# Guanys-dar/GM-Diffusion

Measured on AMD Instinct MI355X. Metric: HDR images/sec @ 512x512, 50 PNDM steps, dual-UNet, higher is better.
Workload: dtype bf16; 1 GPU; SD-v1-5 dual-UNet (SDR 4ch + GM 8ch) 512x512, 50 PNDM steps (51 iterations), CFG 7.5, batch 4/GPU, 2 VAE decodes + Eq.1 HDR tail; global_batch=4, per_gpu_batch=4, resolution=512, inference_steps=50, parallelism=prompt-batch sharding x1, RCCL broadcast of text hidden states + latents

## Files before the change

gm-diffusion_amd/csrc/attention.hip:

```cpp
#include "gmd_common.h"

#include <type_traits>

int gmd_launch_attention_split(const void* Q, const void* K, const void* Vt, void* O, int B, int H, int D, int Nq, int Nk, int64_t ldq,
                               int64_t ldk, int64_t ldvt, int64_t ldo, int64_t sQ, int64_t sK, int64_t sVt, int64_t sO, float scale, int o_split,
                               hipStream_t stream);

namespace {

struct AttnParams {
    const bf16_t* Q;
    const bf16_t* K;
    const bf16_t* Vt;
    bf16_t* O;
    int Nq, Nk, H;
    int64_t ldq, ldk, ldvt, ldo, sQ, sK, sVt, sO;
    float scale_log2;
};

typedef unsigned int u32x4 __attribute__((ext_vector_type(4)));

constexpr int KV = 64;
constexpr int VROW = 136;
constexpr float kNegBig = -1.0e30f;

template <typename HT, int D, bool CAUSAL>
__global__ __launch_bounds__(256, D <= 40 ? 4 : (D <= 64 ? 3 : 1)) void attn_fwd_kernel(const AttnParams p) {
    GMD_WG_TRACE_SCOPE(WGK_ATTN);
    constexpr int DK = (D + 15) / 16;
    constexpr int DT = (D + 31) / 32;
    constexpr int KROW = (2 * DK + 1) * 16;
    constexpr int DC = D / 8;
    static_assert(D % 8 == 0, "head dim must be a multiple of 8");
    extern __shared__ __attribute__((aligned(16))) unsigned char smem[];
    constexpr int kStageBytes = KV * KROW + DT * 32 * VROW;
    constexpr int NKC = (KV * DC + 255) / 256;
    constexpr int NVC = (D * 8 + 255) / 256;
    constexpr bool kRowSumMfma = DT * 32 > D;
    constexpr bool kLagged = kRowSumMfma && DK * 16 > D;
    constexpr float kLagMax = std::is_same<HT, f16_t>::value ? 14.0f : 20.0f;

    const int tid = threadIdx.x, lane = tid & 63, wid = tid >> 6;
    const int r = lane & 31, hh = lane >> 5;
    int qb, head, b;
    {
        const int nwg = gridDim.x, id = blockIdx.x;
        const int qq = nwg >> 3, rr = nwg & 7, xcd = id & 7, j = id >> 3;
        const int L = (xcd < rr ? xcd * (qq + 1) : rr * (qq + 1) + (xcd - rr) * qq) + j;
        const int nqb = (p.Nq + 127) / 128;
        qb = L % nqb;
        const int t = L / nqb;
        head = t % p.H;
        b = t / p.H;
    }
// ... 270 lines not shown
        for (int kt = 0; kt < ntiles; kt += 2) {
            tile(kt, std::integral_constant<int, 0>{}, std::false_type{});
            if (kt + 1 < ntiles) tile(kt + 1, std::integral_constant<int, 1>{}, std::false_type{});
        }
    }

    float l_tot;
    if constexpr (kRowSumMfma) {
        l_tot = __shfl(ot[D / 32][4 * ((D % 32) / 8)], r, 64);
    } else {
        l_tot = half_swap_sum(l_run);
    }
    const float inv = 1.0f / l_tot;
    constexpr int SROW = D * 2 + 16;
    unsigned char* strip = smem + wid * (32 * SROW);
#pragma unroll
    for (int dt = 0; dt < DT; ++dt)
#pragma unroll
        for (int g = 0; g < 4; ++g) {
            const int d0 = 32 * dt + 8 * g + 4 * hh;
            if (d0 < D) {
                uint2 w;
                w.x = Half<HT>::pack2(ot[dt][4 * g + 0] * inv, ot[dt][4 * g + 1] * inv);
                w.y = Half<HT>::pack2(ot[dt][4 * g + 2] * inv, ot[dt][4 * g + 3] * inv);
                *reinterpret_cast<uint2*>(strip + r * SROW + d0 * 2) = w;
            }
        }
    __builtin_amdgcn_wave_barrier();
    constexpr int CH = D / 8;
    const int q0w = qb * 128 + wid * 32;
    bf16_t* Ow = p.O + (int64_t)b * p.sO + (int64_t)q0w * p.ldo + (int64_t)head * D;
#pragma unroll
    for (int t = 0; t < (32 * CH + 63) / 64; ++t) {
        const int idx = lane + 64 * t;
        const int rr = idx / CH, cc = idx - rr * CH;
        if (rr < 32 && q0w + rr < p.Nq)
            *reinterpret_cast<uint4*>(Ow + (int64_t)rr * p.ldo + cc * 8) = *reinterpret_cast<const uint4*>(strip + rr * SROW + cc * 16);
    }
}

template <int N> __device__ __forceinline__ void attn_wait_vmcnt() { asm volatile("s_waitcnt vmcnt(%0)" ::"n"(N) : "memory"); }

#if defined(GMD_ATTN40_PRIO) && GMD_ATTN40_PRIO == 1
#define ATTN40_PRIO_MFMA(x) __builtin_amdgcn_s_setprio(x);
#define ATTN40_PRIO_VALU(x)
#elif defined(GMD_ATTN40_PRIO) && GMD_ATTN40_PRIO == 2
#define ATTN40_PRIO_MFMA(x)
#define ATTN40_PRIO_VALU(x) __builtin_amdgcn_s_setprio(x);
#else
#define ATTN40_PRIO_MFMA(x)
#define ATTN40_PRIO_VALU(x)
#endif
template <typename HT>
__global__ __launch_bounds__(256, 4) void attn40_kernel(const AttnParams p) {
    GMD_WG_TRACE_SCOPE(WGK_ATTN40);
    constexpr int D = 40, DK = 3, DT = 2, NST = 3;
    constexpr int KROWB = 2 * D;
    constexpr int kLagOff = KV * KROWB;
    constexpr int kVOff = 5376;
    constexpr int kStage = kVOff + (D + 2) * 128;
    static_assert(kLagOff + 16 <= kVOff && kStage % 256 == 0, "stage layout");
    constexpr float kLagMax = std::is_same<HT, f16_t>::value ? 14.0f : 20.0f;
    extern __shared__ __attribute__((aligned(16))) unsigned char smem[];

    const int tid = threadIdx.x, lane = tid & 63, wid = tid >> 6;
    const int wuni = __builtin_amdgcn_readfirstlane(wid);
    const int r = lane & 31, hh = lane >> 5;
    int qb, head, b;
    {
        const int nwg = gridDim.x, id = blockIdx.x;
        const int qq = nwg >> 3, rr = nwg & 7, xcd = id & 7, j = id >> 3;
        const int L = (xcd < rr ? xcd * (qq + 1) : rr * (qq + 1) + (xcd - rr) * qq) + j;
        const int nqb = (p.Nq + 127) / 128;
        qb = L % nqb;
        const int t = L / nqb;
        head = t % p.H;
        b = t / p.H;
    }
    const int q = qb * 128 + wid * 32 + r;
    const bool qvalid = q < p.Nq;
    const bf16_t* Qb = p.Q + (int64_t)b * p.sQ + (int64_t)head * D;
    const bf16_t* Kb = p.K + (int64_t)b * p.sK + (int64_t)head * D;
    const bf16_t* Vb = p.Vt + (int64_t)b * p.sVt + (int64_t)head * D * p.ldvt;

    for (int i = tid; i < NST * 24; i += 256) {
        const int st = i / 24, e = i - st * 24;
        unsigned char* base = smem + st * kStage;
        if (e < 8) {
            const unsigned one2 = Half<HT>::kOne | (Half<HT>::kOne << 16);
            *reinterpret_cast<uint4*>(base + kVOff + D * 128 + e * 16) = make_uint4(one2, one2, one2, one2);
        } else if (e < 16) {
            *reinterpret_cast<uint4*>(base + kVOff + (D + 1) * 128 + (e - 8) * 16) = make_uint4(0, 0, 0, 0);
        } else if (e == 16) {
            *reinterpret_cast<uint4*>(base + kLagOff) = make_uint4(Half<HT>::kOne, 0, 0, 0);
        }
    }

    uint4 qf[DK];
#pragma unroll
    for (int s = 0; s < DK; ++s) {
        const int d0 = 16 * s + 8 * hh;
        uint4 v = make_uint4(0, 0, 0, 0);
        if (qvalid && d0 + 8 <= D) v = *reinterpret_cast<const uint4*>(Qb + (int64_t)q * p.ldq + d0);
        unsigned w[4] = {v.x, v.y, v.z, v.w};
#pragma unroll
        for (int j = 0; j < 4; ++j) {
            float lo, hi;
// ... 211 lines not shown
                }
            }
            mx = half_swap_max(mx);
            set_stabiliser(Half<HT>::round(mx));
        }
        for (int kt = 0; kt < ntiles; kt += 3) {
            tile(kt, std::integral_constant<int, 0>{}, lag_c);
            if (kt + 1 < ntiles) tile(kt + 1, std::integral_constant<int, 1>{}, lag_c);
            if (kt + 2 < ntiles) tile(kt + 2, std::integral_constant<int, 2>{}, lag_c);
        }
    };
    run(std::true_type{});
    if (__syncthreads_or(lag_overflow)) {
#pragma unroll
        for (int t = 0; t < DT; ++t)
#pragma unroll
            for (int i = 0; i < 16; ++i) ot[t][i] = 0.f;
        set_stabiliser(0.f);
        m_run = kNegBig;
        run(std::false_type{});
        __syncthreads();
    }

    const float l_tot = __shfl(ot[1][4], r, 64);
    const float inv = 1.0f / l_tot;
    constexpr int SROW = D * 2 + 16;
    unsigned char* strip = smem + wid * (32 * SROW);
#pragma unroll
    for (int dt = 0; dt < DT; ++dt)
#pragma unroll
        for (int g = 0; g < 4; ++g) {
            const int d0 = 32 * dt + 8 * g + 4 * hh;
            if (d0 < D) {
                uint2 w;
                w.x = Half<HT>::pack2(ot[dt][4 * g + 0] * inv, ot[dt][4 * g + 1] * inv);
                w.y = Half<HT>::pack2(ot[dt][4 * g + 2] * inv, ot[dt][4 * g + 3] * inv);
                *reinterpret_cast<uint2*>(strip + r * SROW + d0 * 2) = w;
            }
        }
    __builtin_amdgcn_wave_barrier();
    constexpr int CH = D / 8;
    const int q0w = qb * 128 + wid * 32;
    bf16_t* Ow = p.O + (int64_t)b * p.sO + (int64_t)q0w * p.ldo + (int64_t)head * D;
#pragma unroll
    for (int t = 0; t < (32 * CH + 63) / 64; ++t) {
        const int idx = lane + 64 * t;
        const int rr = idx / CH, cc = idx - rr * CH;
        if (rr < 32 && q0w + rr < p.Nq)
            *reinterpret_cast<uint4*>(Ow + (int64_t)rr * p.ldo + cc * 8) = *reinterpret_cast<const uint4*>(strip + rr * SROW + cc * 16);
    }
}

template <typename HT>
int launch_attn40(const AttnParams& p, int B, int H, hipStream_t s) {
    constexpr size_t smem = 3 * (5376 + 42 * 128);
    dim3 grid(((p.Nq + 127) / 128) * H * B, 1, 1);
    attn40_kernel<HT><<<grid, 256, smem, s>>>(p);
    hipError_t e = hipGetLastError();
    if (e != hipSuccess) {
        gmd_set_error("gmd_attention: launch failed: %s", hipGetErrorString(e));
        return GMD_ERR_LAUNCH;
    }
    return GMD_OK;
}

template <typename HT, int D, bool CAUSAL = false>
int launch_attn(const AttnParams& p, int B, int H, hipStream_t s) {
    constexpr int DK = (D + 15) / 16, DT = (D + 31) / 32;
    const size_t smem = 2 * ((size_t)KV * (2 * DK + 1) * 16 + (size_t)DT * 32 * VROW);
    dim3 grid(((p.Nq + 127) / 128) * H * B, 1, 1);
    attn_fwd_kernel<HT, D, CAUSAL><<<grid, 256, smem, s>>>(p);
    hipError_t e = hipGetLastError();
    if (e != hipSuccess) {
        gmd_set_error("gmd_attention: launch failed: %s", hipGetErrorString(e));
        return GMD_ERR_LAUNCH;
    }
    return GMD_OK;
}

template <typename HT>
int dispatch_attn(const AttnParams& p, int B, int H, int D, int Nq, int Nk, int causal, hipStream_t s) {
    if (causal) {
        GMD_REQUIRE(Nq == Nk, "gmd_attention: the causal mask needs Nq == Nk");
        if (D == 64) return launch_attn<HT, 64, true>(p, B, H, s);
        if (D == 32) return launch_attn<HT, 32, true>(p, B, H, s);
        gmd_set_error("gmd_attention: causal attention is instantiated for head dims 32 and 64 only (got %d)", D);
        return GMD_ERR_UNSUPPORTED;
    }
    switch (D) {
        case 32: return launch_attn<HT, 32>(p, B, H, s);
        case 40: return launch_attn40<HT>(p, B, H, s);
        case 64: return launch_attn<HT, 64>(p, B, H, s);
        case 80: return launch_attn<HT, 80>(p, B, H, s);
        case 160: return launch_attn<HT, 160>(p, B, H, s);
        default:
            gmd_set_error("gmd_attention: head dim %d not instantiated (supported: 32, 40, 64, 80, 160)", D);
            return GMD_ERR_UNSUPPORTED;
    }
}

}

extern "C" int gmd_attention(const void* Q, const void* K, const void* Vt, void* O, int dtype, int B, int H, int D, int Nq,
                             int Nk, int64_t ldq, int64_t ldk, int64_t ldvt, int64_t ldo, int64_t strideQ, int64_t strideK,
                             int64_t strideVt, int64_t strideO, float scale, int causal, gmd_stream_t stream) {
    if (dtype == GMD_F32S || dtype == GMD_F32SA) {
        GMD_REQUIRE(!causal, "gmd_attention: the float32 (split) kernel has no causal mask");
        GMD_REQUIRE(B >= 0 && H > 0 && Nq >= 0 && Nk > 0, "gmd_attention: bad shape B=%d H=%d Nq=%d Nk=%d", B, H, Nq, Nk);
        if (B == 0 || Nq == 0) return GMD_OK;
        GMD_REQUIRE((int64_t)((Nq + 127) / 128) * H * B < (1ll << 31), "gmd_attention: grid too large");
// ... 37 lines not shown
```

gm-diffusion_amd/csrc/gemm.hip:

```cpp
#include "gemm_shared.h"
#include <stdlib.h>
#include <type_traits>

int gmd_launch_split_gemm(const void* params, int presplit, int batch, void* ws, int64_t ws_bytes, hipStream_t s, const char* name);
int gmd_launch_split_conv(const void* params, int presplit, int B, void* ws, int64_t ws_bytes, hipStream_t s, const char* name);
int gmd_split_plan_ksplit(int M, int N, int K, int64_t ws_bytes);
int gmd_split_colstats_ok(int M, int N, int K, int batch, int64_t ws_bytes, int bucket);
int gmd_split_out_ok(int M, int N, int K, int geglu, int64_t ws_bytes);
int gmd_split_qkv_vt_ok(int M, int N, int K, int vt_col0, int vt_tokens, int64_t ws_bytes);
void gmd_split_set_lc(int mode);

namespace {

template <typename HT>
__device__ __forceinline__ void epilogue_store8(const GemmParams& p, int z, int m, int n, float (&v)[8]) {
    const bool vec_ok = (p.ldc % 8 == 0) && (p.sC % 8 == 0) && (p.residual == nullptr || (p.ldr % 8 == 0 && p.sR % 8 == 0));
    const int nvalid = p.N - n < 8 ? p.N - n : 8;
    const float* rb = p.rowbias ? p.rowbias + (int64_t)(m / p.rows_per_group) * p.ldrb : nullptr;
    const HT* res = p.residual ? (const HT*)p.residual + (int64_t)z * p.sR + (int64_t)m * p.ldr + n : nullptr;
    float rv[8];
    if (res) {
        if (nvalid == 8 && vec_ok) load_vec(res, rv);
        else
            for (int j = 0; j < 8; ++j) rv[j] = j < nvalid ? Elem<HT>::ld(res + j) : 0.f;
// ... 882 lines not shown
            wait_tiles(rem < D - 1 ? rem : D - 1);
            __syncthreads();
            if (kt + D < nk) dma_tile(kt + D, st_fill);
            compute(st_cur);
            st_cur = st_cur + 1 == NST ? 0 : st_cur + 1;
            st_fill = st_fill + 1 == NST ? 0 : st_fill + 1;
        }
    }
    const bool rows_ok = !p.out_f32 && p.ksplit <= 1 && p.act != GMD_ACT_GEGLU && m0 + BM <= p.M && n0 + BN <= p.N && (p.ldc & 7) == 0 &&
                         (p.sC & 7) == 0 && (p.residual == nullptr || ((p.ldr & 7) == 0 && (p.sR & 7) == 0)) &&
                         (p.rowbias == nullptr || ((p.ldrb & 3) == 0 && (reinterpret_cast<uintptr_t>(p.rowbias) & 15) == 0)) &&
                         (reinterpret_cast<uintptr_t>(p.bias) & 15) == 0;
    if constexpr (TN % 2 == 0) {
        if (p.act == GMD_ACT_GEGLU && !p.out_f32 && p.ksplit <= 1 && m0 + BM <= p.M && n0 + BN <= p.N && (p.ldc & 7) == 0 && (p.sC & 7) == 0 &&
            (reinterpret_cast<uintptr_t>(p.bias) & 15) == 0) {
            __syncthreads();
            constexpr int kStripG = 32 * (TN * 8 + 4);
            epilogue_rows_geglu<HT, TM, TN>(p, acc, reinterpret_cast<float*>(smem) + wid * kStripG, m0 + wr * 64, n0 + wc * (TN * 16), lane, z);
            return;
        }
    }
    if (p.ksplit > 1 && m0 + BM <= p.M && n0 + BN <= p.N && (p.N & 3) == 0) {
        __syncthreads();
        constexpr int kStripS = 32 * (TN * 16 + 4);
        epilogue_rows_slab<TM, TN>(p, acc, reinterpret_cast<float*>(smem) + wid * kStripS, m0 + wr * 64, n0 + wc * (TN * 16), lane, ks);
        return;
    }
    if (__builtin_expect(rows_ok, 1)) {
        __syncthreads();
        constexpr int kStrip = 32 * (TN * 16 + 4);
        static_assert((size_t)NWAVES * kStrip * 4 <= (size_t)NST * kStage, "epilogue strips must fit in the ring stages");
        epilogue_rows<HT, TM, TN>(p, acc, reinterpret_cast<float*>(smem) + wid * kStrip, m0 + wr * 64, n0 + wc * (TN * 16), lane, z);
    } else {
        epilogue_regs<HT, TM, TN>(p, acc, m0 + wr * 64, n0 + wc * (TN * 16), frow, fq, z, ks);
    }
}

template <typename HT, bool CONV, int TN>
__global__ __launch_bounds__(768, 3) void gemm_pp_kernel(const GemmParams p) {
    GMD_WG_TRACE_SCOPE(WGK_PP | (CONV ? WGK_CONV_BIT : 0));
    constexpr int WN = 2, NCONS = 8, LW = 4, TM = 4, NST = 3;
    constexpr int BM = 256, BN = WN * TN * 16;
    constexpr int RPP = LW * 8;
    constexpr int NA = BM / RPP;
    constexpr int NW = BN / RPP;
    constexpr int NP = NA + NW;
    static_assert(BN % RPP == 0, "W tile rows must be whole staging passes");
    extern __shared__ __attribute__((aligned(16))) unsigned char smem[];
    constexpr int kStage = (BM + BN) * 128;

    const int tid = threadIdx.x, lane = tid & 63, wid = tid >> 6;
    const int wuni = __builtin_amdgcn_readfirstlane(wid);
    const bool loader = wuni >= NCONS;
    const bool late = wuni >= 4 && !loader;
    int m0, n0;
    {
        const int nwg = gridDim.x, id = blockIdx.x;
        const int q = nwg >> 3, r = nwg & 7, xcd = id & 7, j = id >> 3;
        const int L = (xcd < r ? xcd * (q + 1) : r * (q + 1) + (xcd - r) * q) + j;
        const int tiles_n = (p.N + BN - 1) / BN, tiles_m = (p.M + BM - 1) / BM;
        int mt, nt;
        grouped_tile(L, tiles_m, tiles_n, p.tile_group, mt, nt);
        m0 = mt * BM;
        n0 = nt * BN;
    }
    const int z = p.ksplit > 1 ? 0 : blockIdx.z;
    const int ks = p.ksplit > 1 ? blockIdx.z : 0;
    const int nk_total = p.K / BK;
    const int per = (nk_total + p.ksplit - 1) / p.ksplit;
    const int kt_begin = ks * per;
    const int nk = (kt_begin + per <= nk_total ? per : nk_total - kt_begin);

    auto seg_barrier = [&]() {
        __builtin_amdgcn_sched_barrier(0);
        __builtin_amdgcn_s_barrier();
        __builtin_amdgcn_sched_barrier(0);
    };
#ifdef GMD_PP_DIAG
    unsigned long long dg[8] = {0, 0, 0, 0, 0, 0, 0, 0}, dprev = 0, dreal0 = 0, dtime0 = 0;
    auto stamp_now = [&]() {
        unsigned long long t;
        __builtin_amdgcn_sched_barrier(0);
        asm volatile("s_memtime %0\n\ts_waitcnt lgkmcnt(0)" : "=s"(t)::"memory");
        __builtin_amdgcn_sched_barrier(0);
        return t;
    };
    auto diag_begin = [&]() {
        dprev = stamp_now();
        dtime0 = dprev;
        asm volatile("s_memrealtime %0\n\ts_waitcnt lgkmcnt(0)" : "=s"(dreal0)::"memory");
    };
    auto diag_end = [&]() {
        unsigned long long dreal1;
        asm volatile("s_memrealtime %0\n\ts_waitcnt lgkmcnt(0)" : "=s"(dreal1)::"memory");
        dg[7] = dreal1 - dreal0;
#ifdef GMD_WG_TRACE
        if (lane == 0 && g_wg_trace != nullptr) {
            GmdWgTraceHeader* h = g_wg_trace;
            const unsigned hw = __builtin_amdgcn_s_getreg((31 << 11) | 4), xcc = __builtin_amdgcn_s_getreg((31 << 11) | 20);
            const unsigned shard = ((((xcc & 7u) * 8u + ((hw >> 13) & 7u)) * 2u + ((hw >> 12) & 1u)) * 16u) + ((hw >> 8) & 15u);
            unsigned long long* counters = reinterpret_cast<unsigned long long*>(h + 1);
            const unsigned long long i = __hip_atomic_fetch_add(counters + 16ull * shard, 1ull, __ATOMIC_RELAXED, __HIP_MEMORY_SCOPE_WORKGROUP);
            if (i < h->capacity) {
                uint4* rec = reinterpret_cast<uint4*>(counters + 16ull * h->shards) + 2ull * (shard * h->capacity + i);
                const unsigned a0 = (unsigned)(loader ? dg[1] : dg[0]), a1 = (unsigned)dg[3], a2 = (unsigned)(loader ? 0 : dg[4]), a3 = (unsigned)(loader ? dg[6] : dg[5]);
                rec[0] = make_uint4(a0, a1, a2, a3);
                rec[1] = make_uint4(hw, (xcc & 15u) | ((unsigned)((WGK_PP | (CONV ? WGK_CONV_BIT : 0)) | 0x80) << 8) | ((unsigned)wid << 16), (unsigned)nk | ((unsigned)TN << 16),
// ... 77 lines not shown
            asm volatile("s_mov_b32 m0, %1\n\ts_nop 0\n\tbuffer_load_dwordx4 %0, %2, %3 offen lds"
                         :
                         : "v"(voff), "s"(lds_addr), "s"(desc), "s"(soff)
                         : "memory", "m0");
#pragma clang diagnostic pop
        };
        auto dma_part = [&](auto QC, int kt, int stage_idx) {
            constexpr int Q = decltype(QC)::value;
            constexpr int lo = Q == 4 ? 0 : Q * NP / 4, hi = Q == 4 ? NP : (Q + 1) * NP / 4;
            unsigned kbytes = (unsigned)(kt_begin + kt) * (BK * 2);
            unsigned abytes = kbytes;
            if (CONV) {
                if ((Q == 0 || Q == 4) && newtap) {
                    const int ky = tap / 3, kx = tap - ky * 3;
#pragma unroll
                    for (int i = 0; i < NA; ++i) aoff[i] = conv_tap_offset<CONV>(p, pv[i], pb[i], py[i], px[i], ky, kx, chunk);
                    newtap = false;
                }
                abytes = (unsigned)c0 * 2u;
                kbytes = (unsigned)(tap * p.Cin + c0) * 2u;
            }
            const unsigned stage = lds_base + (unsigned)stage_idx * kStage + (unsigned)lw * (8 * 128);
#pragma unroll
            for (int i = 0; i < NA; ++i)
                if (i >= lo && i < hi) dma16(dA, stage + i * (RPP * 128), aoff[i], abytes);
#pragma unroll
            for (int i = 0; i < NW; ++i)
                if (NA + i >= lo && NA + i < hi) dma16(dW, stage + BM * 128 + i * (RPP * 128), woff[i], kbytes);
            if (CONV && (Q == 3 || Q == 4)) {
                c0 += BK;
                if (c0 >= cb0 + p.cblk) {
                    c0 = cb0;
                    ++tap;
                    newtap = true;
                    if (tap == 9) { tap = 0; cb0 += p.cblk; c0 = cb0; }
                }
            }
        };
        if (nk > 0) {
            dma_part(IntC<4>{}, 0, 0);
            if (nk > 1) {
                dma_part(IntC<4>{}, 1, 1);
                wait_vmcnt<NP>();
            } else {
                wait_vmcnt<0>();
            }
            seg_barrier();
            int st_fill = 2;
#ifdef GMD_PP_DIAG
            diag_begin();
#endif
            for (int kt = 0; kt < nk; ++kt) {
                const bool more = kt + 2 < nk;
                if (more) dma_part(IntC<0>{}, kt + 2, st_fill);
                PP_STAMP(1)
                seg_barrier();
                PP_STAMP(3)
                if (more) dma_part(IntC<1>{}, kt + 2, st_fill);
                PP_STAMP(1)
                seg_barrier();
                PP_STAMP(3)
                if (more) dma_part(IntC<2>{}, kt + 2, st_fill);
                PP_STAMP(1)
                seg_barrier();
                PP_STAMP(3)
                if (more) dma_part(IntC<3>{}, kt + 2, st_fill);
                PP_STAMP(1)
                if (more) wait_vmcnt<NP>();
                else wait_vmcnt<0>();
                PP_STAMP(6)
                seg_barrier();
                PP_STAMP(3)
                st_fill = st_fill == NST - 1 ? 0 : st_fill + 1;
            }
#ifdef GMD_PP_DIAG
            diag_end();
#endif
            seg_barrier();
        }
        __syncthreads();
        return;
    }

    const int wr = wid / WN, wc = wid % WN;
    f32x4 acc[TM][TN];
#pragma unroll
    for (int i = 0; i < TM; ++i)
#pragma unroll
        for (int j = 0; j < TN; ++j) acc[i][j] = f32x4{0.f, 0.f, 0.f, 0.f};
    const int frow = lane & 15, fq = lane >> 4;
    uint4 fa[TM], fb[TN];
    auto frag_reads = [&](int stage_idx, int s2) {
        const unsigned char* sA = smem + stage_idx * kStage;
        const unsigned char* sW = sA + BM * 128;
#pragma unroll
        for (int i = 0; i < TM; ++i) fa[i] = *reinterpret_cast<const uint4*>(sA + lds_off(wr * 64 + i * 16 + frow, 4 * s2 + fq));
#pragma unroll
        for (int j = 0; j < TN; ++j) fb[j] = *reinterpret_cast<const uint4*>(sW + lds_off(wc * (TN * 16) + j * 16 + frow, 4 * s2 + fq));
    };
    auto mfmas = [&]() {
#pragma unroll
        for (int i = 0; i < TM; ++i)
#pragma unroll
            for (int j = 0; j < TN; ++j) acc[i][j] = Half<HT>::mfma16(fb[j], fa[i], acc[i][j]);
    };
    auto lgkm0 = [&]() { asm volatile("s_waitcnt lgkmcnt(0)" ::: "memory"); };

    if (nk > 0) {
        seg_barrier();
        if (late) seg_barrier();
        int st = 0;
#ifdef GMD_PP_DIAG
        diag_begin();
#endif
        for (int kt = 0; kt < nk; ++kt) {
#pragma unroll
            for (int s2 = 0; s2 < 2; ++s2) {
                frag_reads(st, s2);
                lgkm0();
                PP_STAMP(0)
                seg_barrier();
                PP_STAMP(3)
                __builtin_amdgcn_s_setprio(1);
                mfmas();
                __builtin_amdgcn_s_setprio(0);
                PP_STAMP(4)
                seg_barrier();
                PP_STAMP(5)
            }
            st = st == NST - 1 ? 0 : st + 1;
        }
#ifdef GMD_PP_DIAG
        diag_end();
#endif
        if (!late) seg_barrier();
    }
#if defined(GMD_PP_DIAG) && defined(GMD_WG_TRACE)
    unsigned long long ph_sync = 0;
    auto real_now = [&]() { unsigned long long t; asm volatile("s_memrealtime %0\n\ts_waitcnt lgkmcnt(0)" : "=s"(t)::"memory"); return t; };
    auto phase_emit = [&]() {
        if (wid != 0 || lane != 0 || g_wg_trace == nullptr || nk <= 0) return;
        const unsigned long long t_end = real_now();
        GmdWgTraceHeader* h = g_wg_trace;
        const unsigned hw = __builtin_amdgcn_s_getreg((31 << 11) | 4), xcc = __builtin_amdgcn_s_getreg((31 << 11) | 20);
        const unsigned shard = ((((xcc & 7u) * 8u + ((hw >> 13) & 7u)) * 2u + ((hw >> 12) & 1u)) * 16u) + ((hw >> 8) & 15u);
        unsigned long long* counters = reinterpret_cast<unsigned long long*>(h + 1);
        const unsigned long long i2 = __hip_atomic_fetch_add(counters + 16ull * shard, 1ull, __ATOMIC_RELAXED, __HIP_MEMORY_SCOPE_WORKGROUP);
        if (i2 < h->capacity) {
            uint4* rec = reinterpret_cast<uint4*>(counters + 16ull * h->shards) + 2ull * (shard * h->capacity + i2);
            rec[0] = make_uint4((unsigned)(dreal0 - gmd_wg_trace_scope_.t0), (unsigned)dg[7], (unsigned)(ph_sync - (dreal0 + dg[7])), (unsigned)(t_end - ph_sync));
            rec[1] = make_uint4(hw, (xcc & 15u) | ((unsigned)((WGK_PP | (CONV ? WGK_CONV_BIT : 0)) | 0x80) << 8) | (0xFFu << 16), (unsigned)nk | ((unsigned)TN << 16),
                                (gridDim.x * gridDim.z) | ((unsigned)p.ksplit << 20) | (p.residual ? (1u << 28) : 0u) | (p.fixup ? (1u << 29) : 0u));
        }
    };
#define PP_PHASE_SYNC() ph_sync = real_now()
#define PP_PHASE_EMIT() phase_emit()
#else
#define PP_PHASE_SYNC()
#define PP_PHASE_EMIT()
#endif
    __syncthreads();
    GemmParams q = p;
    if (p.fixup) {
        if (!splitk_fixup<TM, TN, NCONS>(p, acc, ks, wid, lane)) return;
        q.ksplit = 1;
    }
    PP_PHASE_SYNC();
    const bool rows_ok = !q.out_f32 && q.ksplit <= 1 && q.act != GMD_ACT_GEGLU && m0 + BM <= q.M && n0 + BN <= q.N && (q.ldc & 7) == 0 &&
                         (q.sC & 7) == 0 && (q.residual == nullptr || ((q.ldr & 7) == 0 && (q.sR & 7) == 0)) &&
                         (q.rowbias == nullptr || ((q.ldrb & 3) == 0 && (reinterpret_cast<uintptr_t>(q.rowbias) & 15) == 0)) &&
                         (reinterpret_cast<uintptr_t>(q.bias) & 15) == 0;
    if constexpr (TN % 2 == 0) {
        if (q.act == GMD_ACT_GEGLU && !q.out_f32 && q.ksplit <= 1 && m0 + BM <= q.M && n0 + BN <= q.N && (q.ldc & 7) == 0 && (q.sC & 7) == 0 &&
            (reinterpret_cast<uintptr_t>(q.bias) & 15) == 0) {
            constexpr int kStripG = 32 * (TN * 8 + 4);
            epilogue_rows_geglu<HT, TM, TN>(q, acc, reinterpret_cast<float*>(smem) + wid * kStripG, m0 + wr * 64, n0 + wc * (TN * 16), lane, z);
            PP_PHASE_EMIT();
            return;
        }
    }
    if (__builtin_expect(q.ksplit > 1 && m0 + BM <= q.M && n0 + BN <= q.N && (q.N & 3) == 0, 0)) {
        constexpr int kStripS = 32 * (TN * 16 + 4);
        epilogue_rows_slab<TM, TN>(q, acc, reinterpret_cast<float*>(smem) + wid * kStripS, m0 + wr * 64, n0 + wc * (TN * 16), lane, ks);
        PP_PHASE_EMIT();
        return;
    }
    if (__builtin_expect(rows_ok, 1)) {
        constexpr int kStrip = 32 * (TN * 16 + 4);
// ... 1397 lines not shown
```

Baseline: 5.395 HDR images/s.

## Rework D=40 attention LDS layout into V^T pieces with shared ones comb

Adds a new attn40 kernel that reorganises the per-stage shared-memory layout: V^T is split into 1152-byte pieces per 8-row group, a constant 'comb' of ones feeds the row-sum MFMA lanes, and the K/V DMA work is redistributed across waves (3 pieces for waves 0-1, 2 for waves 2-3). Partial tiles are masked in LDS, and the stage size grows to 11776 bytes. The intent is to reduce LDS bank conflicts and balance async-load issue across waves. The old kernel is kept, selectable through an environment variable. The larger stage size may affect occupancy.

```diff
diff --git a/gm-diffusion_amd/csrc/attention.hip b/gm-diffusion_amd/csrc/attention.hip
--- a/gm-diffusion_amd/csrc/attention.hip
+++ b/gm-diffusion_amd/csrc/attention.hip
@@ -1,5 +1,7 @@
 #include "gmd_common.h"
 
+#include <cstdlib>
+#include <cstring>
 #include <type_traits>
 
 int gmd_launch_attention_split(const void* Q, const void* K, const void* Vt, void* O, int B, int H, int D, int Nq, int Nk, int64_t ldq,
@@ -376,7 +378,7 @@
 #define ATTN40_PRIO_VALU(x)
 #endif
 template <typename HT>
-__global__ __launch_bounds__(256, 4) void attn40_kernel(const AttnParams p) {
+__global__ __launch_bounds__(256, 4) void attn40_kernel_r5(const AttnParams p) {
     GMD_WG_TRACE_SCOPE(WGK_ATTN40);
     constexpr int D = 40, DK = 3, DT = 2, NST = 3;
     constexpr int KROWB = 2 * D;
@@ -694,10 +696,336 @@
 }
 
 template <typename HT>
+__global__ __launch_bounds__(256, 4) void attn40_kernel(const AttnParams p) {
+    GMD_WG_TRACE_SCOPE(WGK_ATTN40);
+    constexpr int D = 40, DK = 3, DT = 2, NST = 3;
+    constexpr int KROWB = 2 * D;
+    constexpr int kVOff = KV * KROWB;
+    constexpr int kVPiece = 1152;
+    constexpr int kComb = kVOff + 4 * kVPiece + 1024;
+    constexpr int kLagOff = kComb + 16;
+    constexpr int kStage = 11776;
+    static_assert((kComb - kVOff - 4 * kVPiece) % 256 == 0, "the comb shares the bank pattern of the d = 32..39 piece");
+    static_assert(kComb + 3 * 256 + 128 + 16 <= kStage && kStage % 256 == 0, "stage layout");
+    constexpr float kLagMax = std::is_same<HT, f16_t>::value ? 14.0f : 20.0f;
+    extern __shared__ __attribute__((aligned(16))) unsigned char smem[];
+
+    const int tid = threadIdx.x, lane = tid & 63, wid = tid >> 6;
+    const int wuni = __builtin_amdgcn_readfirstlane(wid);
+    const int r = lane & 31, hh = lane >> 5;
+    int qb, head, b;
+    {
+        const int nwg = gridDim.x, id = blockIdx.x;
+        const int qq = nwg >> 3, rr = nwg & 7, xcd = id & 7, j = id >> 3;
+        const int L = (xcd < rr ? xcd * (qq + 1) : rr * (qq + 1) + (xcd - rr) * qq) + j;
+        const int nqb = (p.Nq + 127) / 128;
+        qb = L % nqb;
+        const int t = L / nqb;
+        head = t % p.H;
+        b = t / p.H;
+    }
+    const int q = qb * 128 + wid * 32 + r;
+    const bool qvalid = q < p.Nq;
+    const bf16_t* Qb = p.Q + (int64_t)b * p.sQ + (int64_t)head * D;
+    const bf16_t* Kb = p.K + (int64_t)b * p.sK + (int64_t)head * D;
+    const bf16_t* Vb = p.Vt + (int64_t)b * p.sVt + (int64_t)head * D * p.ldvt;
+
+    if (tid < NST * 9) {
+        const int st = tid / 9, e = tid - st * 9;
+        unsigned char* base = smem + st * kStage;
+        const unsigned one2 = Half<HT>::kOne | (Half<HT>::kOne << 16);
+        if (e < 8) *reinterpret_cast<uint4*>(base + kComb + (e >> 1) * 256 + (e & 1) * 128) = make_uint4(one2, one2, one2, one2);
+        else *reinterpret_cast<uint4*>(base + kLagOff) = make_uint4(Half<HT>::kOne, 0, 0, 0);
+    }
+
+    uint4 qf[DK];
+#pragma unroll
+    for (int s = 0; s < DK; ++s) {
+        const int d0 = 16 * s + 8 * hh;
+        uint4 v = make_uint4(0, 0, 0, 0);
+        if (qvalid && d0 + 8 <= D) v = *reinterpret_cast<const uint4*>(Qb + (int64_t)q * p.ldq + d0);
+        unsigned w[4] = {v.x, v.y, v.z, v.w};
+#pragma unroll
+        for (int j = 0; j < 4; ++j) {
+            float lo, hi;
+            Half<HT>::unpack2(w[j], lo, hi);
+            w[j] = Half<HT>::pack2(lo * p.scale_log2, hi * p.scale_log2);
+        }
+        qf[s] = make_uint4(w[0], w[1], w[2], w[3]);
+    }
+    f32x16 ot[DT];
+#pragma unroll
+    for (int t = 0; t < DT; ++t)
+#pragma unroll
+        for (int i = 0; i < 16; ++i) ot[t][i] = 0.f;
+    float m_run = 0.f;
+    int lag_max = 0;
+    const unsigned stab_sel = hh ? 0x0c0c0706u : 0x03020100u;
+    auto stabiliser_bits = [&](float t) { return Half<HT>::pack2(t, -t); };
+    auto low_half = [&](unsigned bits) { float lo, hi; Half<HT>::unpack2(bits, lo, hi); return lo; };
+    auto set_stabiliser = [&](unsigned bits) {
+        m_run = low_half(bits);
+        qf[2].x = __builtin_amdgcn_perm(bits, qf[2].x, stab_sel);
+    };
+
+    const int kr = (r & ~12) | ((r & 4) << 1) | ((r & 8) >> 1);
+    const int kb = kr * KROWB + hh * 16;
+    const int kl0 = hh ? kLagOff : kr * KROWB + 64;
+    const int kl1 = hh ? kLagOff : (32 + kr) * KROWB + 64;
+    const int vb0 = kVOff + (r >> 3) * kVPiece + (8 * hh + (r & 7)) * 16;
+    const int vb1 = r < 8 ? kVOff + 4 * kVPiece + (8 * hh + r) * 16 : kComb + (hh ? 0 : 128);
+
+    constexpr int kPiecesW01 = 3, kPiecesW23 = 2;
+    static_assert((2 * kPiecesW01 + 2 * kPiecesW23) * 64 == KV * (D / 8) + D * (KV / 8), "every 16-byte chunk of a K / V^T tile is one lane of one piece");
+    const unsigned lds_base = __builtin_amdgcn_readfirstlane((unsigned)(size_t)(__attribute__((address_space(3))) void*)smem);
+    u32x4 dK, dV;
+    {
+        const uint64_t bk = (uint64_t)Kb, bv = (uint64_t)Vb;
+        const unsigned kbytes = (unsigned)((((int64_t)p.Nk - 1) * p.ldk + D) * 2);
+        const unsigned vbytes = (unsigned)((((int64_t)D - 1) * p.ldvt + (p.Nk + 7) / 8 * 8) * 2);
+        dK = u32x4{(unsigned)__builtin_amdgcn_readfirstlane((unsigned)bk), (unsigned)__builtin_amdgcn_readfirstlane((unsigned)(bk >> 32) & 0xffffu),
+                   (unsigned)__builtin_amdgcn_readfirstlane(kbytes), 0x00020000u};
+        dV = u32x4{(unsigned)__builtin_amdgcn_readfirstlane((unsigned)bv), (unsigned)__builtin_amdgcn_readfirstlane((unsigned)(bv >> 32) & 0xffffu),
+                   (unsigned)__builtin_amdgcn_readfirstlane(vbytes), 0x00020000u};
+    }
+    auto k_src = [&](int g) { const int key = g / 5, c = g - key * 5; return (unsigned)(key * (int)p.ldk + c * 8) * 2u; };
+    auto v_src = [&](int i, int l) { return (unsigned)((8 * i + (l & 7)) * (int)p.ldvt + (l >> 3) * 8) * 2u; };
+    const unsigned off0 = k_src(tid);
+    const unsigned off1 = wuni == 0 ? k_src(tid + 256) : v_src(wuni - 1, lane);
+    const unsigned off2 = v_src(3 + (wuni & 1), lane);
+    const unsigned dst0 = (unsigned)wuni * 1024u;
+    const unsigned dst1 = wuni == 0 ? 4096u : (unsigned)(kVOff + (wuni - 1) * kVPiece);
+    const unsigned dst2 = (unsigned)(kVOff + (3 + (wuni & 1)) * kVPiece);
+    auto dma16 = [&](const u32x4& desc, unsigned lds_addr, unsigned voff, unsigned soff) {
+#pragma clang diagnostic push
+#pragma clang diagnostic ignored "-Winline-asm"
+        asm volatile("s_mov_b32 m0, %1\n\ts_nop 0\n\tbuffer_load_dwordx4 %0, %2, %3 offen lds"
+                     :
+                     : "v"(voff), "s"(lds_addr), "s"(desc), "s"(soff)
+                     : "memory", "m0");
+#pragma clang diagnostic pop
+    };
+    const int ntiles = (p.Nk + KV - 1) / KV;
+    auto pieces = [&](unsigned sb, unsigned a0, unsigned a1, unsigned a2, unsigned ks_off, unsigned vs_off) {
+        dma16(dK, sb + dst0, a0, ks_off);
+        if (wuni == 0) dma16(dK, sb + dst1, a1, ks_off);
+        else dma16(dV, sb + dst1, a1, vs_off);
+        if (wuni < 2) dma16(dV, sb + dst2, a2, vs_off);
+    };
+    auto issue = [&](int kt, int stage) {
+        const int k0 = kt * KV;
+        const unsigned ks_off = (unsigned)k0 * (unsigned)p.ldk * 2u, vs_off = (unsigned)k0 * 2u;
+        const unsigned sb = lds_base + (unsigned)stage * kStage;
+        if (k0 + KV <= p.Nk) pieces(sb, off0, off1, off2, ks_off, vs_off);
+        else
+            pieces(sb, off0 + ks_off, off1 + (wuni == 0 ? ks_off : vs_off), off2 + vs_off, 0u, 0u);
+    };
+    auto wait_tile = [&](bool more) {
+        if (!more) attn_wait_vmcnt<0>();
+        else if (wuni < 2) attn_wait_vmcnt<kPiecesW01>();
+        else attn_wait_vmcnt<kPiecesW23>();
+    };
+    auto first_product = [&](const unsigned char* Sb, int t) {
+        f32x16 acc;
+#pragma unroll
+        for (int i = 0; i < 16; ++i) acc[i] = 0.f;
+#pragma unroll
+        for (int s = 0; s < 2; ++s)
+            acc = Half<HT>::mfma32(*reinterpret_cast<const uint4*>(Sb + kb + t * (32 * KROWB) + 32 * s), qf[s], acc);
+        return Half<HT>::mfma32(*reinterpret_cast<const uint4*>(Sb + (t ? kl1 : kl0)), qf[2], acc);
+    };
+    auto max_nonneg = [](float a, float b) { return __int_as_float(max(__float_as_int(a), __float_as_int(b))); };
+
+    auto tile = [&](const int kt, auto stage_c, auto lag_c, auto steady_c) {
+        constexpr bool LAG = decltype(lag_c)::value;
+        constexpr int STAGE = decltype(stage_c)::value;
+        constexpr bool STEADY = decltype(steady_c)::value;
+        const int k0 = kt * KV;
+        if constexpr (STEADY) wait_tile(true);
+        else wait_tile(kt + 1 < ntiles);
+        __syncthreads();
+        const unsigned char* Sb = smem + STAGE * kStage;
+        const bool partial = !STEADY && k0 + KV > p.Nk;
+        if (partial) {
+            for (int id = tid; id < D * 8; id += 256) {
+                const int c = (id & 63) >> 3;
+                const int nv = p.Nk - (k0 + c * 8);
+                if (nv < 8) {
+                    uint4* cell = reinterpret_cast<uint4*>(smem + STAGE * kStage + kVOff + (id >> 6) * kVPiece + (id & 63) * 16);
+                    const uint4 x = *cell;
+                    unsigned w[4] = {x.x, x.y, x.z, x.w};
+#pragma unroll
+                    for (int e = 0; e < 4; ++e) {
+                        if (2 * e >= nv) w[e] = 0;
+                        else if (2 * e + 1 >= nv) w[e] &= 0xffffu;
+                    }
+                    *cell = make_uint4(w[0], w[1], w[2], w[3]);
+                }
+            }
+            __syncthreads();
+        }
+        if (STEADY || kt + 2 < ntiles) issue(kt + 2, (STAGE + 2) % NST);
+
+        f32x16 st[2];
+#pragma unroll
+        for (int t = 0; t < 2; ++t) st[t] = first_product(Sb, t);
+        if (partial) {
+#pragma unroll
+            for (int t = 0; t < 2; ++t)
+#pragma unroll
+                for (int i = 0; i < 16; ++i) {
+                    const int key = k0 + 32 * t + 16 * (i >> 3) + 8 * hh + (i & 7);
+                    if (key >= p.Nk) st[t][i] = kNegBig;
+                }
+        }
+        uint4 pf[4];
+        if constexpr (LAG) {
+            float mx = 0.f;
+#pragma unroll
+            for (int i = 0; i < 16; ++i) mx = fmaxf(fmaxf(mx, st[0][i]), st[1][i]);
+            {
+                const auto sw = __builtin_amdgcn_permlane32_swap(__float_as_uint(mx), __float_as_uint(mx), false, false);
+                mx = max_nonneg(__uint_as_float(sw[0]), __uint_as_float(sw[1]));
+            }
+            lag_max = max(lag_max, __float_as_int(mx));
+#pragma unroll
+            for (int t = 0; t < 2; ++t)
+#pragma unroll
+                for (int i = 0; i < 16; ++i) st[t][i] = __builtin_amdgcn_exp2f(st[t][i]);
+#pragma unroll
+            for (int t = 0; t < 2; ++t)
+#pragma unroll
+                for (int s = 0; s < 2; ++s)
+                    pf[2 * t + s] = make_uint4(Half<HT>::pack2(st[t][8 * s + 0], st[t][8 * s + 1]), Half<HT>::pack2(st[t][8 * s + 2], st[t][8 * s + 3]),
+                                               Half<HT>::pack2(st[t][8 * s + 4], st[t][8 * s + 5]), Half<HT>::pack2(st[t][8 * s + 6], st[t][8 * s + 7]));
+            const unsigned bits = stabiliser_bits(m_run + mx);
+            const float m_new = low_half(bits);
+#pragma unroll
+            for (int ks = 0; ks < 4; ++ks) {
+                ot[0] = Half<HT>::mfma32(*reinterpret_cast<const uint4*>(Sb + vb0 + 256 * ks), pf[ks], ot[0]);
+                ot[1] = Half<HT>::mfma32(*reinterpret_cast<const uint4*>(Sb + vb1 + 256 * ks), pf[ks], ot[1]);
+            }
+            if (!__all(m_new == m_run)) {
+                const float alpha = __builtin_amdgcn_exp2f(m_run - m_new);
+#pragma unroll
+                for (int t = 0; t < DT; ++t)
+#pragma unroll
+                    for (int i = 0; i < 16; ++i) ot[t][i] *= alpha;
+                set_stabiliser(bits);
+            }
+        } else {
+            float mx = fmaxf(st[0][0], st[1][0]);
+#pragma unroll
+            for (int i = 1; i < 16; ++i) mx = fmaxf(fmaxf(mx, st[0][i]), st[1][i]);
+            mx = half_swap_max(mx);
+            const float m_new = fmaxf(m_run, mx);
+            const float alpha = __builtin_amdgcn_exp2f(m_run - m_new);
+            m_run = m_new;
+#pragma unroll
+            for (int t = 0; t < 2; ++t)
+#pragma unroll
+                for (int i = 0; i < 16; ++i) st[t][i] = __builtin_amdgcn_exp2f(st[t][i] - m_new);
+            if (!__all(alpha == 1.0f)) {
+#pragma unroll
+                for (int t = 0; t < DT; ++t)
+#pragma unroll
+                    for (int i = 0; i < 16; ++i) ot[t][i] *= alpha;
+            }
+#pragma unroll
+            for (int t = 0; t < 2; ++t)
+#pragma unroll
+                for (int s = 0; s < 2; ++s)
+                    pf[2 * t + s] = make_uint4(Half<HT>::pack2(st[t][8 * s + 0], st[t][8 * s + 1]), Half<HT>::pack2(st[t][8 * s + 2], st[t][8 * s + 3]),
+                                               Half<HT>::pack2(st[t][8 * s + 4], st[t][8 * s + 5]), Half<HT>::pack2(st[t][8 * s + 6], st[t][8 * s + 7]));
+#pragma unroll
+            for (int ks = 0; ks < 4; ++ks) {
+                ot[0] = Half<HT>::mfma32(*reinterpret_cast<const uint4*>(Sb + vb0 + 256 * ks), pf[ks], ot[0]);
+                ot[1] = Half<HT>::mfma32(*reinterpret_cast<const uint4*>(Sb + vb1 + 256 * ks), pf[ks], ot[1]);
+            }
+        }
+    };
+    auto run = [&](auto lag_c) {
+        constexpr bool LAG = decltype(lag_c)::value;
+        using S0 = std::integral_constant<int, 0>;
+        using S1 = std::integral_constant<int, 1>;
+        using S2 = std::integral_constant<int, 2>;
+        issue(0, 0);
+        if (ntiles > 1) issue(1, 1);
+        if constexpr (LAG) {
+            wait_tile(ntiles > 1);
+            __syncthreads();
+            float mx = kNegBig;
+#pragma unroll
+            for (int t = 0; t < 2; ++t) {
+                const f32x16 s0 = first_product(smem, t);
+#pragma unroll
+                for (int i = 0; i < 16; ++i) {
+                    const int key = 32 * t + 16 * (i >> 3) + 8 * hh + (i & 7);
+                    if (key < p.Nk) mx = fmaxf(mx, s0[i]);
+                }
+            }
+            mx = half_swap_max(mx);
+            set_stabiliser(stabiliser_bits(mx));
+        }
+        int kt = 0;
+        for (; kt + 5 <= ntiles; kt += 3) {
+            tile(kt, S0{}, lag_c, std::true_type{});
+            tile(kt + 1, S1{}, lag_c, std::true_type{});
+            tile(kt + 2, S2{}, lag_c, std::true_type{});
+        }
+        for (; kt < ntiles; kt += 3) {
+            tile(kt, S0{}, lag_c, std::false_type{});
+            if (kt + 1 < ntiles) tile(kt + 1, S1{}, lag_c, std::false_type{});
+            if (kt + 2 < ntiles) tile(kt + 2, S2{}, lag_c, std::false_type{});
+        }
+    };
+    run(std::true_type{});
+    if (__syncthreads_or(__int_as_float(lag_max) > kLagMax)) {
+#pragma unroll
+        for (int t = 0; t < DT; ++t)
+#pragma unroll
+            for (int i = 0; i < 16; ++i) ot[t][i] = 0.f;
+        set_stabiliser(stabiliser_bits(0.f));
+        m_run = kNegBig;
+        run(std::false_type{});
+        __syncthreads();
+    }
+
+    const float l_tot = __shfl(ot[1][4], r, 64);
+    const float inv = 1.0f / l_tot;
+    constexpr int SROW = D * 2 + 16;
+    unsigned char* strip = smem + wid * (32 * SROW);
+#pragma unroll
+    for (int dt = 0; dt < DT; ++dt)
+#pragma unroll
+        for (int g = 0; g < 4; ++g) {
+            const int d0 = 32 * dt + 8 * g + 4 * hh;
+            if (d0 < D) {
+                uint2 w;
+                w.x = Half<HT>::pack2(ot[dt][4 * g + 0] * inv, ot[dt][4 * g + 1] * inv);
+                w.y = Half<HT>::pack2(ot[dt][4 * g + 2] * inv, ot[dt][4 * g + 3] * inv);
+                *reinterpret_cast<uint2*>(strip + r * SROW + d0 * 2) = w;
+            }
+        }
+    __builtin_amdgcn_wave_barrier();
+    constexpr int CH = D / 8;
+    const int q0w = qb * 128 + wid * 32;
+    bf16_t* Ow = p.O + (int64_t)b * p.sO + (int64_t)q0w * p.ldo + (int64_t)head * D;
+#pragma unroll
+    for (int t = 0; t < (32 * CH + 63) / 64; ++t) {
+        const int idx = lane + 64 * t;
+        const int rr = idx / CH, cc = idx - rr * CH;
+        if (rr < 32 && q0w + rr < p.Nq)
+            *reinterpret_cast<uint4*>(Ow + (int64_t)rr * p.ldo + cc * 8) = *reinterpret_cast<const uint4*>(strip + rr * SROW + cc * 16);
+    }
+}
+
+template <typename HT>
 int launch_attn40(const AttnParams& p, int B, int H, hipStream_t s) {
-    constexpr size_t smem = 3 * (5376 + 42 * 128);
     dim3 grid(((p.Nq + 127) / 128) * H * B, 1, 1);
-    attn40_kernel<HT><<<grid, 256, smem, s>>>(p);
+    const char* knob = getenv("GMD_ATTN40");
+    if (knob && strcmp(knob, "r5") == 0) attn40_kernel_r5<HT><<<grid, 256, 3 * (5376 + 42 * 128), s>>>(p);
+    else attn40_kernel<HT><<<grid, 256, 3 * 11776, s>>>(p);
     hipError_t e = hipGetLastError();
     if (e != hipSuccess) {
         gmd_set_error("gmd_attention: launch failed: %s", hipGetErrorString(e));
```

New measurement: 5.450 HDR images/s (median of 6 runs). 1.01x the previous value.

## Collapse producer/consumer GEMM pipeline to one barrier per k-tile

Applied to the files above, without the earlier changes.

The loader waves in the warp-specialized pingpong GEMM now issue each stage's full DMA at once instead of four parts separated by barriers. Consumer waves read both k-halves' fragments up front, run both MFMA groups back to back, and meet at a single barrier per k-tile. The late/early wave staggering and its extra barriers are removed. This cuts barrier count and sync stalls in the main loop, at the cost of doubled fragment registers and burstier global-load issue, and it drops the staggered overlap between the two consumer halves.

```diff
diff --git a/gm-diffusion_amd/csrc/gemm.hip b/gm-diffusion_amd/csrc/gemm.hip
--- a/gm-diffusion_amd/csrc/gemm.hip
+++ b/gm-diffusion_amd/csrc/gemm.hip
@@ -958,7 +958,6 @@
     const int tid = threadIdx.x, lane = tid & 63, wid = tid >> 6;
     const int wuni = __builtin_amdgcn_readfirstlane(wid);
     const bool loader = wuni >= NCONS;
-    const bool late = wuni >= 4 && !loader;
     int m0, n0;
     {
         const int nwg = gridDim.x, id = blockIdx.x;
@@ -1142,19 +1141,7 @@
 #endif
             for (int kt = 0; kt < nk; ++kt) {
                 const bool more = kt + 2 < nk;
-                if (more) dma_part(IntC<0>{}, kt + 2, st_fill);
-                PP_STAMP(1)
-                seg_barrier();
-                PP_STAMP(3)
-                if (more) dma_part(IntC<1>{}, kt + 2, st_fill);
-                PP_STAMP(1)
-                seg_barrier();
-                PP_STAMP(3)
-                if (more) dma_part(IntC<2>{}, kt + 2, st_fill);
-                PP_STAMP(1)
-                seg_barrier();
-                PP_STAMP(3)
-                if (more) dma_part(IntC<3>{}, kt + 2, st_fill);
+                if (more) dma_part(IntC<4>{}, kt + 2, st_fill);
                 PP_STAMP(1)
                 if (more) wait_vmcnt<NP>();
                 else wait_vmcnt<0>();
@@ -1166,7 +1153,6 @@
 #ifdef GMD_PP_DIAG
             diag_end();
 #endif
-            seg_barrier();
         }
         __syncthreads();
         return;
@@ -1179,8 +1165,8 @@
 #pragma unroll
         for (int j = 0; j < TN; ++j) acc[i][j] = f32x4{0.f, 0.f, 0.f, 0.f};
     const int frow = lane & 15, fq = lane >> 4;
-    uint4 fa[TM], fb[TN];
-    auto frag_reads = [&](int stage_idx, int s2) {
+    uint4 fa0[TM], fb0[TN], fa1[TM], fb1[TN];
+    auto frag_reads = [&](int stage_idx, int s2, uint4 (&fa)[TM], uint4 (&fb)[TN]) {
         const unsigned char* sA = smem + stage_idx * kStage;
         const unsigned char* sW = sA + BM * 128;
 #pragma unroll
@@ -1188,42 +1174,38 @@
 #pragma unroll
         for (int j = 0; j < TN; ++j) fb[j] = *reinterpret_cast<const uint4*>(sW + lds_off(wc * (TN * 16) + j * 16 + frow, 4 * s2 + fq));
     };
-    auto mfmas = [&]() {
+    auto mfmas = [&](const uint4 (&fa)[TM], const uint4 (&fb)[TN]) {
+        __builtin_amdgcn_s_setprio(1);
 #pragma unroll
         for (int i = 0; i < TM; ++i)
 #pragma unroll
             for (int j = 0; j < TN; ++j) acc[i][j] = Half<HT>::mfma16(fb[j], fa[i], acc[i][j]);
+        __builtin_amdgcn_s_setprio(0);
     };
-    auto lgkm0 = [&]() { asm volatile("s_waitcnt lgkmcnt(0)" ::: "memory"); };
 
     if (nk > 0) {
         seg_barrier();
-        if (late) seg_barrier();
         int st = 0;
 #ifdef GMD_PP_DIAG
         diag_begin();
 #endif
         for (int kt = 0; kt < nk; ++kt) {
-#pragma unroll
-            for (int s2 = 0; s2 < 2; ++s2) {
-                frag_reads(st, s2);
-                lgkm0();
-                PP_STAMP(0)
-                seg_barrier();
-                PP_STAMP(3)
-                __builtin_amdgcn_s_setprio(1);
-                mfmas();
-                __builtin_amdgcn_s_setprio(0);
-                PP_STAMP(4)
-                seg_barrier();
-                PP_STAMP(5)
-            }
+            frag_reads(st, 0, fa0, fb0);
+            frag_reads(st, 1, fa1, fb1);
+            PP_STAMP(0)
+            __builtin_amdgcn_sched_barrier(0);
+            mfmas(fa0, fb0);
+            __builtin_amdgcn_sched_barrier(0);
+            mfmas(fa1, fb1);
+            asm volatile("s_waitcnt lgkmcnt(0)" ::: "memory");
+            PP_STAMP(4)
+            seg_barrier();
+            PP_STAMP(5)
             st = st == NST - 1 ? 0 : st + 1;
         }
 #ifdef GMD_PP_DIAG
         diag_end();
 #endif
-        if (!late) seg_barrier();
     }
 #if defined(GMD_PP_DIAG) && defined(GMD_WG_TRACE)
     unsigned long long ph_sync = 0;
```

After: 5.308 HDR images/s before, 5.183 HDR images/s after (median of 2 runs). -2.4%, worse.
